# rpacheco-blazquez/PINN-FEM

Measured on AMD Instinct MI355X. Metric: element-residual-grad evals/sec (PINN+GD iteration: MLP fwd+bwd, stiffness, assembly, residual, Adam), collinear truss, higher is better.
Workload: dtype f32; 1 GPU; ex4 shape (nets (20, 15, 10), E and A evaluated), 1000000 elements per GPU, collinear 2-D truss h=1, alpha_data=100 with measurements at every node, load factor 0.1; elements_total=1000000, parallelism=elements sharded x1

## Files before the change

### include/pinnfem_hip.h

```cpp
#ifndef PINNFEM_HIP_H
#define PINNFEM_HIP_H

#include <stdint.h>

#ifdef __cplusplus
extern "C" {
#endif

#define PF_ABI_VERSION 7

#define PF_OK 0
#define PF_ERR_ARG (-1)
#define PF_ERR_UNSUPPORTED (-2)
#define PF_ERR_HIP (-3)

#define PF_DOF_FIXED 1u
#define PF_DOF_MEASURED 2u
#define PF_DOF_SHARED 4u
#define PF_DOF_GHOST 8u

#define PF_WG_SHUFFLE 0
#define PF_WG_MFMA 1
#define PF_WG_MFMA44 2
#define PF_WG_MFMA32 3
// ... 60 lines not shown
  int32_t n_tensors;
  int32_t wg_mode;
  float lam;
  float alpha_physics, alpha_data;
  float lr_u, lr_t;
  double tol;
  double beta1, beta2, eps;
  int32_t use_data;
  int32_t max_iter;
  float* theta_pad;
  float* prop_e;
  float* prop_a;
  float* g_f;
  float* g_ea;
  float* grad_u;
  float* grad_theta;
  float* partials;
  float* hist;
  pf_state* state;
  int32_t n_part_blocks;
  int32_t pad_total;
  const int32_t* pad_index;
  float n_meas_f;
  int32_t fe_mode;
  const int32_t* shared_dofs;
  const int32_t* shared_slot;
  int32_t n_shared;
  int32_t n_iface;
  int32_t own_lo, own_hi;
  int32_t part_half;
  int32_t prop_double;
  float* net_op;
  int32_t op_off[2];
  int32_t coord_exp;
  int32_t mlp_dtype;
  float* elem_k;
  float* theta_alt;
  float* u_alt;
  const int32_t* adj_other;
} pf_problem;

#define PF_MAX_BLOCKS 1024
#define PF_MAX_NODE_BLOCKS 4096
#define PF_NODE_SLOTS (PF_MAX_NODE_BLOCKS + 8)

int pf_abi_version(void);
const char* pf_last_error(void);
int pf_net_param_count(int in_dim, int width, int n_hidden);
int pf_padded_width(int width);
int pf_net_pad_count(int in_dim, int width, int n_hidden);
int pf_net_pad_index(int in_dim, int width, int n_hidden, int local);
int pf_sizeof(int what);
int pf_net_op_count(int in_dim, int width, int n_hidden);
long long pf_partials_count(const pf_problem* p);
#define PF_FUSED_FORWARD 1
#define PF_FUSED_BACKWARD 2
#define PF_FUSED_THETA_UPDATE 4
#define PF_FUSED_U_PINGPONG 8
#define PF_FUSED_U_UPDATE 16
int pf_fusion_info(const pf_problem* p);

int pf_pack_theta(const pf_problem* p, void* stream);
int pf_net_forward(const pf_problem* p, int which, void* stream);
int pf_net_forward_all(const pf_problem* p, void* stream);
int pf_net_backward_all(const pf_problem* p, void* stream);
int pf_internal_force(const pf_problem* p, const float* u, float* f_int_out, void* stream);
int pf_node_residual(const pf_problem* p, float* f_int_out, void* stream);
int pf_elem_adjoint(const pf_problem* p, void* stream);
int pf_net_backward(const pf_problem* p, int which, void* stream);
int pf_node_gradu(const pf_problem* p, int fuse_adam, void* stream);
int pf_theta_reduce(const pf_problem* p, int fuse_adam, void* stream);
int pf_finalize(const pf_problem* p, void* stream);
int pf_reset(const pf_problem* p, void* stream);

int pf_gd_iterations(const pf_problem* p, int n_iter, void* stream);
int pf_graph_create(const pf_problem* p, int iters_per_graph, void* stream, void** graph_out);
#define PF_GRAPH_CONT_HEAD 1
#define PF_GRAPH_NO_TAIL 2
int pf_graph_create_ex(const pf_problem* p, int iters_per_graph, int flags, void* stream, void** graph_out);
int pf_graph_tail(const pf_problem* p, int iters_per_graph, void* stream);
int pf_graph_launch(void* graph, void* stream);
int pf_graph_destroy(void* graph);
#define PF_KERNEL_SLOTS 9
int pf_gd_iterations_timed(const pf_problem* p, int n_iter, void* stream, float* ms_per_kernel);
int pf_loss_and_grads(const pf_problem* p, void* stream);

int pf_shard_forward(const pf_problem* p, void* stream);
int pf_shard_backward(const pf_problem* p, float* buf, const float* u2_local, void* stream);
int pf_shard_update_interior(const pf_problem* p, void* stream);
int pf_shard_update_shared(const pf_problem* p, const float* buf, float* u2_local, void* stream);
int pf_shard_flush(const pf_problem* p, const float* u2_reduced, void* stream);

#define PF_COMM_ID_BYTES 128
int pf_comm_unique_id(const char* librccl_path, void* id_out);
int pf_comm_create(const char* librccl_path, const void* id, int rank, int world, void** comm_out);
int pf_comm_destroy(void* comm);
int pf_comm_abort(void* comm);
int pf_comm_info(void* comm, int* rank_out, int* nranks_out);
int pf_comm_all_reduce(void* comm, float* buf, int n, void* stream);
int pf_shard_iterations(const pf_problem* p, void* comm, int n_iter, float* buf, float* u2_local, void* stream);
int pf_shard_graph_create(const pf_problem* p, void* comm, int iters_per_graph, float* buf, float* u2_local, void* stream,
                          void** graph_out);
int pf_shard_iterations_graph(const pf_problem* p, void* comm, void* graph, int iters_per_graph, int n_iter, float* buf,
                              float* u2_local, void* stream);

int pf_kv_f64(const pf_problem* p, const double* v, double* out, int zero_fixed, void* stream);
// ... 32 lines not shown
```

### pinn_fem_amd/_capi.py

```python
from __future__ import annotations

import ctypes as C
import os

_HERE = os.path.dirname(os.path.abspath(__file__))
LIB_PATH = os.environ.get("PINNFEM_LIB") or os.path.join(_HERE, "lib", "libpinnfem_hip.so")

PF_ABI_VERSION = 7
PF_OK, PF_ERR_ARG, PF_ERR_UNSUPPORTED, PF_ERR_HIP = 0, -1, -2, -3
PF_DOF_FIXED, PF_DOF_MEASURED, PF_DOF_SHARED, PF_DOF_GHOST = 1, 2, 4, 8
PF_WG_SHUFFLE, PF_WG_MFMA, PF_WG_MFMA44, PF_WG_MFMA32 = 0, 1, 2, 3
PF_N32_WIDTH_MAX = 30
PF_MLP_F32, PF_MLP_BF16 = 0, 1
PF_FE_REFERENCE, PF_FE_DELTA = 0, 1
PF_HIST_COLS = 6
PF_MAX_BLOCKS = 1024
PF_COMM_ID_BYTES = 128
PF_MAX_NODE_BLOCKS = 4096
PF_NODE_SLOTS = PF_MAX_NODE_BLOCKS + 8
PF_KERNEL_SLOTS = 9
PF_GRAPH_CONT_HEAD, PF_GRAPH_NO_TAIL = 1, 2
PF_FUSED_FORWARD, PF_FUSED_BACKWARD, PF_FUSED_THETA_UPDATE, PF_FUSED_U_PINGPONG, PF_FUSED_U_UPDATE = 1, 2, 4, 8, 16
KERNEL_SLOT_NAMES = ("net_forward_young", "net_forward_area", "node_residual", "elem_adjoint",
                     "net_backward_young", "net_backward_area", "node_gradu_adam", "theta_reduce_adam",
# ... 27 lines not shown
        ("_pad2", C.c_float),
        ("loss_total", C.c_float), ("loss_physics", C.c_float), ("loss_data", C.c_float),
        ("u_norm", C.c_float), ("residual_norm", C.c_float), ("theta_norm", C.c_float),
        ("u_half", C.c_int32), ("_pad3", C.c_float),
    ]


class PfProblem(C.Structure):
    _fields_ = [
        ("mesh", PfMesh), ("net", PfNet * 2),
        ("u", C.c_void_p), ("m_u", C.c_void_p), ("v_u", C.c_void_p),
        ("theta", C.c_void_p), ("m_t", C.c_void_p), ("v_t", C.c_void_p),
        ("n_theta", C.c_int32), ("n_theta_active", C.c_int32),
        ("tensor_off", C.c_void_p),
        ("n_tensors", C.c_int32), ("wg_mode", C.c_int32),
        ("lam", C.c_float), ("alpha_physics", C.c_float), ("alpha_data", C.c_float),
        ("lr_u", C.c_float), ("lr_t", C.c_float),
        ("tol", C.c_double), ("beta1", C.c_double), ("beta2", C.c_double), ("eps", C.c_double),
        ("use_data", C.c_int32), ("max_iter", C.c_int32),
        ("theta_pad", C.c_void_p), ("prop_e", C.c_void_p), ("prop_a", C.c_void_p),
        ("g_f", C.c_void_p), ("g_ea", C.c_void_p), ("grad_u", C.c_void_p),
        ("grad_theta", C.c_void_p), ("partials", C.c_void_p), ("hist", C.c_void_p),
        ("state", C.c_void_p),
        ("n_part_blocks", C.c_int32), ("pad_total", C.c_int32),
        ("pad_index", C.c_void_p),
        ("n_meas_f", C.c_float), ("fe_mode", C.c_int32),
        ("shared_dofs", C.c_void_p), ("shared_slot", C.c_void_p),
        ("n_shared", C.c_int32), ("n_iface", C.c_int32),
        ("own_lo", C.c_int32), ("own_hi", C.c_int32), ("part_half", C.c_int32), ("prop_double", C.c_int32),
        ("net_op", C.c_void_p), ("op_off", C.c_int32 * 2), ("coord_exp", C.c_int32), ("mlp_dtype", C.c_int32),
        ("elem_k", C.c_void_p), ("theta_alt", C.c_void_p), ("u_alt", C.c_void_p), ("adj_other", C.c_void_p),
    ]


class PfScalarId(C.Structure):
    _fields_ = [
        ("p", C.c_void_p), ("m_p", C.c_void_p), ("v_p", C.c_void_p), ("table", C.c_void_p),
        ("n_rows", C.c_int32), ("has_bounds", C.c_int32),
        ("lo", C.c_float * 2), ("hi", C.c_float * 2),
        ("inv_ea0", C.c_float), ("lr_p", C.c_float), ("n_free_f", C.c_float), ("_pad", C.c_float),
    ]


_PP = C.POINTER(PfProblem)
SYMBOLS = {
    "pf_abi_version": (C.c_int, []),
    "pf_last_error": (C.c_char_p, []),
    "pf_net_param_count": (C.c_int, [C.c_int, C.c_int, C.c_int]),
    "pf_padded_width": (C.c_int, [C.c_int]),
    "pf_net_pad_count": (C.c_int, [C.c_int, C.c_int, C.c_int]),
    "pf_net_pad_index": (C.c_int, [C.c_int, C.c_int, C.c_int, C.c_int]),
    "pf_sizeof": (C.c_int, [C.c_int]),
    "pf_net_op_count": (C.c_int, [C.c_int, C.c_int, C.c_int]),
    "pf_partials_count": (C.c_longlong, [_PP]),
    "pf_fusion_info": (C.c_int, [_PP]),
    "pf_pack_theta": (C.c_int, [_PP, C.c_void_p]),
    "pf_net_forward": (C.c_int, [_PP, C.c_int, C.c_void_p]),
    "pf_net_forward_all": (C.c_int, [_PP, C.c_void_p]),
    "pf_net_backward_all": (C.c_int, [_PP, C.c_void_p]),
    "pf_internal_force": (C.c_int, [_PP, C.c_void_p, C.c_void_p, C.c_void_p]),
    "pf_node_residual": (C.c_int, [_PP, C.c_void_p, C.c_void_p]),
    "pf_elem_adjoint": (C.c_int, [_PP, C.c_void_p]),
    "pf_net_backward": (C.c_int, [_PP, C.c_int, C.c_void_p]),
    "pf_node_gradu": (C.c_int, [_PP, C.c_int, C.c_void_p]),
    "pf_theta_reduce": (C.c_int, [_PP, C.c_int, C.c_void_p]),
    "pf_finalize": (C.c_int, [_PP, C.c_void_p]),
    "pf_reset": (C.c_int, [_PP, C.c_void_p]),
    "pf_gd_iterations": (C.c_int, [_PP, C.c_int, C.c_void_p]),
    "pf_graph_create": (C.c_int, [_PP, C.c_int, C.c_void_p, C.POINTER(C.c_void_p)]),
    "pf_graph_create_ex": (C.c_int, [_PP, C.c_int, C.c_int, C.c_void_p, C.POINTER(C.c_void_p)]),
    "pf_graph_tail": (C.c_int, [_PP, C.c_int, C.c_void_p]),
    "pf_graph_launch": (C.c_int, [C.c_void_p, C.c_void_p]),
    "pf_graph_destroy": (C.c_int, [C.c_void_p]),
    "pf_gd_iterations_timed": (C.c_int, [_PP, C.c_int, C.c_void_p, C.POINTER(C.c_float)]),
    "pf_loss_and_grads": (C.c_int, [_PP, C.c_void_p]),
    "pf_shard_forward": (C.c_int, [_PP, C.c_void_p]),
    "pf_shard_backward": (C.c_int, [_PP, C.c_void_p, C.c_void_p, C.c_void_p]),
    "pf_shard_flush": (C.c_int, [_PP, C.c_void_p, C.c_void_p]),
    "pf_shard_update_interior": (C.c_int, [_PP, C.c_void_p]),
    "pf_shard_update_shared": (C.c_int, [_PP, C.c_void_p, C.c_void_p, C.c_void_p]),
    "pf_kv_f64": (C.c_int, [_PP, C.c_void_p, C.c_void_p, C.c_int, C.c_void_p]),
    "pf_pcg_workspace_count": (C.c_longlong, [_PP]),
    "pf_pcg_begin": (C.c_int, [_PP, C.c_void_p, C.c_void_p, C.c_void_p, C.c_double, C.c_void_p]),
    "pf_pcg_iterations": (C.c_int, [_PP, C.c_void_p, C.c_void_p, C.c_int, C.POINTER(C.c_double), C.c_void_p]),
    "pf_pcg_graph_create": (C.c_int, [_PP, C.c_void_p, C.c_void_p, C.c_int, C.c_void_p, C.POINTER(C.c_void_p)]),
    "pf_pcg_state": (C.c_int, [_PP, C.c_void_p, C.POINTER(C.c_double), C.c_void_p]),
    "pf_comm_unique_id": (C.c_int, [C.c_char_p, C.c_void_p]),
    "pf_comm_create": (C.c_int, [C.c_char_p, C.c_void_p, C.c_int, C.c_int, C.POINTER(C.c_void_p)]),
    "pf_comm_destroy": (C.c_int, [C.c_void_p]),
    "pf_comm_abort": (C.c_int, [C.c_void_p]),
    "pf_comm_info": (C.c_int, [C.c_void_p, C.POINTER(C.c_int), C.POINTER(C.c_int)]),
    "pf_comm_all_reduce": (C.c_int, [C.c_void_p, C.c_void_p, C.c_int, C.c_void_p]),
    "pf_shard_iterations": (C.c_int, [_PP, C.c_void_p, C.c_int, C.c_void_p, C.c_void_p, C.c_void_p]),
    "pf_shard_graph_create": (C.c_int, [_PP, C.c_void_p, C.c_int, C.c_void_p, C.c_void_p, C.c_void_p,
                                        C.POINTER(C.c_void_p)]),
    "pf_shard_iterations_graph": (C.c_int, [_PP, C.c_void_p, C.c_void_p, C.c_int, C.c_int, C.c_void_p, C.c_void_p,
                                            C.c_void_p]),
    "pf_scalar_gd_iterations": (C.c_int, [_PP, C.POINTER(PfScalarId), C.c_int, C.c_void_p]),
    "pf_adam": (C.c_int, [C.c_void_p, C.c_void_p, C.c_void_p, C.c_void_p, C.c_int, C.c_int,
                          C.c_double, C.c_double, C.c_double, C.c_double, C.c_void_p]),
    "pf_diag_k": (C.c_int, [_PP, C.c_void_p, C.c_void_p]),
    "pf_dense_k": (C.c_int, [_PP, C.c_void_p, C.c_void_p]),
    "pf_coo_k": (C.c_int, [_PP, C.c_void_p, C.c_void_p, C.c_void_p, C.c_void_p]),
}


# ... 50 lines not shown
```

### pinn_fem_amd/csrc/pf_api.hip

```cpp
#include <stdlib.h>
#include <string.h>
#include <stdio.h>
#include "pf_common.h"
#include "pf_net32.h"

int pf_launch_node_residual(const pf_problem* p, float* f_int_out, int compute_loss, hipStream_t s, int fin_prev = 0);
int pf_launch_elem_adjoint(const pf_problem* p, hipStream_t s);
int pf_launch_node_gradu(const pf_problem* p, int fuse_adam, hipStream_t s, int skip_shared = 0, float* u_out = nullptr);
int pf_launch_u_home(const pf_problem* p, hipStream_t s);
int pf_launch_scalar_residual(const pf_problem* p, const pf_scalar_id* sp, hipStream_t s);
int pf_launch_scalar_update(const pf_problem* p, const pf_scalar_id* sp, hipStream_t s);
int pf_launch_shard_pack(const pf_problem* p, float* buf2, const float* u2_local, hipStream_t s);
int pf_launch_shard_update(const pf_problem* p, const float* buf2, float* u2_local, hipStream_t s);
int pf_launch_shard_flush(const pf_problem* p, const float* u2, hipStream_t s);
int pf_launch_theta_reduce(const pf_problem* p, int fuse_adam, hipStream_t s);
int pf_launch_pack_theta(const pf_problem* p, hipStream_t s);
int pf_launch_finalize(const pf_problem* p, int mode, int with_theta, hipStream_t s, int tn_ready = 0);
int pf_launch_theta_stage1(const pf_problem* p, hipStream_t s);
int pf_launch_theta_stage2(const pf_problem* p, int fuse_adam, hipStream_t s);
int pf_launch_reset(const pf_problem* p, hipStream_t s);
int pf_launch_adam(float* param, const float* grad, float* m, float* v, int n, int step, double lr,
                   double beta1, double beta2, double eps, hipStream_t s);
int pf_launch_diag_k(const pf_problem* p, float* diag, hipStream_t s);
int pf_launch_dense_k(const pf_problem* p, float* K, hipStream_t s);
// ... 212 lines not shown

int pf_abi_version(void) { return PF_ABI_VERSION; }
const char* pf_last_error(void) { return g_err; }

int pf_sizeof(int what) {
  switch (what) {
    case 0: return (int)sizeof(pf_mesh);
    case 1: return (int)sizeof(pf_net);
    case 2: return (int)sizeof(pf_state);
    case 3: return (int)sizeof(pf_problem);
    case 4: return (int)sizeof(pf_scalar_id);
  }
  return PF_ERR_ARG;
}

int pf_net_param_count(int in_dim, int width, int n_hidden) {
  if (in_dim < 1 || width < 1 || n_hidden < 1) return PF_ERR_ARG;
  return width * in_dim + width + (n_hidden - 1) * (width * width + width) + width + 1;
}

int pf_padded_width(int width) { return padded_width(width); }

int pf_net_pad_count(int in_dim, int width, int n_hidden) {
  const int hp = padded_width(width);
  if (hp < 0 || n_hidden < 1 || n_hidden > 3 || (in_dim != 2 && in_dim != 3)) return PF_ERR_UNSUPPORTED;
  return pf_pad_count(hp, n_hidden);
}

int pf_net_pad_index(int in_dim, int width, int n_hidden, int local) {
  const int hp = padded_width(width);
  if (hp < 0 || n_hidden < 1 || n_hidden > 3 || (in_dim != 2 && in_dim != 3)) return PF_ERR_UNSUPPORTED;
  int q = local;
  if (q < 0) return PF_ERR_ARG;
  if (q < width * in_dim) return (q / in_dim) * 4 + (q % in_dim);
  q -= width * in_dim;
  if (q < width) return q * 4 + in_dim;
  q -= width;
  for (int l = 2; l <= n_hidden; ++l) {
    if (q < width * width) return pf_pad_wh(hp, l) + (q / width) * (hp + 4) + (q % width);
    q -= width * width;
    if (q < width) return pf_pad_wh(hp, l) + q * (hp + 4) + hp;
    q -= width;
  }
  if (q < width) return pf_pad_wo(hp, n_hidden) + q;
  q -= width;
  if (q == 0) return pf_pad_wo(hp, n_hidden) + hp;
  return PF_ERR_ARG;
}

int pf_net_op_count(int in_dim, int width, int n_hidden) {
  if (width < 1 || width > PF_N32_WIDTH_MAX || n_hidden < 1 || n_hidden > 3 || (in_dim != 2 && in_dim != 3))
    return PF_ERR_UNSUPPORTED;
  return (pf_n32_bytes(n_hidden) + 3) / 4;
}

long long pf_partials_count(const pf_problem* p) {
  if (!p) return PF_ERR_ARG;
  return (long long)PF_PART_WG + ((long long)p->n_part_blocks + PF_RG) * (long long)p->pad_total;
}

int pf_fusion_info(const pf_problem* p) {
  if (check_problem(p) != PF_OK) return PF_ERR_ARG;
  int m = 0;
  if (can_fuse_forward(p)) m |= PF_FUSED_FORWARD;
  if (can_fuse_backward(p)) m |= PF_FUSED_BACKWARD;
  if (can_fuse_theta_update(p)) m |= PF_FUSED_THETA_UPDATE;
  if (p->prop_double != 0 && p->elem_k != nullptr && can_fuse_gradu(p)) m |= PF_FUSED_U_UPDATE;
  else if (p->u_alt != nullptr && p->mesh.n_elems >= PF_GRAPH_DAG_MIN_ELEMS) m |= PF_FUSED_U_PINGPONG;
  return m;
}

int pf_pack_theta(const pf_problem* p, void* stream) {
  int rc = check_problem(p);
  if (rc) return rc;
  PF_TRY(pf_launch_pack_theta(p, (hipStream_t)stream), "pf_pack_theta");
  return PF_OK;
}

int pf_net_forward(const pf_problem* p, int which, void* stream) {
  int rc = check_problem(p);
  if (rc) return rc;
  if (which < 0 || which > 1 || !p->net[which].enabled) return fail(PF_ERR_ARG, "net not enabled");
  PF_TRY(net_forward(p, which, (hipStream_t)stream), "pf_net_forward");
  return PF_OK;
}

int pf_net_forward_all(const pf_problem* p, void* stream) {
  int rc = check_problem(p);
  if (rc) return rc;
  PF_TRY(net_forward_all(p, (hipStream_t)stream), "pf_net_forward_all");
  return PF_OK;
}

int pf_net_backward_all(const pf_problem* p, void* stream) {
  int rc = check_problem(p);
  if (rc) return rc;
  if (!(p->net[0].enabled || p->net[1].enabled)) return PF_OK;
  return enqueue_backwards(p, (hipStream_t)stream);
}

int pf_internal_force(const pf_problem* p, const float* u, float* f_int_out, void* stream) {
  int rc = check_problem(p);
  if (rc) return rc;
  if (!u || !f_int_out) return fail(PF_ERR_ARG, "null u / f_int_out");
  pf_problem q = *p;
  q.u = const_cast<float*>(u);
// ... 502 lines not shown
```

### pinn_fem_amd/csrc/pf_net32.h

```cpp
#pragma once
#include "pf_common.h"

#define PF_N32_MAX_WIDTH 30
#define PF_N32_KA 2048.0f
#define PF_N32_KW 16.0f
#define PF_N32_KB 16.0f
__host__ __device__ inline float pf_n32_lam_scale(float lam) {
  const float a = lam < 0.f ? -lam : lam;
  if (!(a > 0.f) || !(a < 3.0e38f)) return 1.0f;
  int ex = 0;
  (void)frexpf(a, &ex);
  ex = ex < -100 ? -100 : ex;
  return ldexpf(1.0f, 14 - ex);
}

__host__ __device__ constexpr int pf_n32_off_w1() { return 16; }
__host__ __device__ constexpr int pf_n32_off_wo() { return 16 + 512; }
__host__ __device__ constexpr int pf_n32_off_bo() { return 16 + 512 + 128; }
__host__ __device__ constexpr int pf_n32_off_layers() { return 16 + 512 + 128 + 16; }
#define PF_N32_LAYER_BYTES (128 + 4096 + 4096)
__host__ __device__ constexpr int pf_n32_off_bias(int l) { return pf_n32_off_layers() + (l - 2) * PF_N32_LAYER_BYTES; }
__host__ __device__ constexpr int pf_n32_off_af(int l) { return pf_n32_off_bias(l) + 128; }
__host__ __device__ constexpr int pf_n32_off_ab(int l) { return pf_n32_off_af(l) + 4096; }
__host__ __device__ constexpr int pf_n32_bytes(int n_hidden) { return pf_n32_off_layers() + (n_hidden - 1) * PF_N32_LAYER_BYTES; }
// ... 37 lines not shown
      unsigned short hf[8], hb[8];
#pragma unroll
      for (int j = 0; j < 8; ++j) {
        const int u_k = 2 * (8 * ks + j) + hh;
        float vf = 0.f, vb = 0.f;
        if (u_row < W && u_k < W) {
          vf = PF_N32_KW * Wl[u_row * W + u_k];
          vb = PF_N32_KB * Wl[u_k * W + u_row];
        }
        if (prec == 1) {
          hf[j] = sp ? (unsigned short)0 : __builtin_bit_cast(unsigned short, (__bf16)vf);
          hb[j] = sp ? (unsigned short)0 : __builtin_bit_cast(unsigned short, (__bf16)vb);
        } else {
          const _Float16 fh = (_Float16)vf, bh = (_Float16)vb;
          hf[j] = __builtin_bit_cast(unsigned short, sp ? (_Float16)(vf - (float)fh) : fh);
          hb[j] = __builtin_bit_cast(unsigned short, sp ? (_Float16)(vb - (float)bh) : bh);
        }
      }
      af[i] = make_uint4(hf[0] | (unsigned)hf[1] << 16, hf[2] | (unsigned)hf[3] << 16, hf[4] | (unsigned)hf[5] << 16,
                         hf[6] | (unsigned)hf[7] << 16);
      ab[i] = make_uint4(hb[0] | (unsigned)hb[1] << 16, hb[2] | (unsigned)hb[3] << 16, hb[4] | (unsigned)hb[5] << 16,
                         hb[6] | (unsigned)hb[7] << 16);
    }
  }
  if (with_bound && (tid >> 6) == ((nt - 1) >> 6)) {
    const int lane = tid & 63;
    float v = lane < W ? fabsf(th[o_wo + lane]) : 0.f;
    float bound = 0.f, grow = 1.f;
    for (int l = L; l >= 1; --l) {
      float m = v;
#pragma unroll
      for (int d = 32; d >= 1; d >>= 1) m = fmaxf(m, __shfl_xor(m, d));
      bound = fmaxf(bound, grow * m);
      grow *= 4.f;
      if (l >= 2) {
        const float* Wl = th + o_h + (l - 2) * per;
        float a = 0.f;
#pragma unroll 4
        for (int j = 0; j < W; ++j) {
          const float w = lane < W ? fabsf(Wl[j * W + lane]) : 0.f;
          a += w * __shfl(v, j);
        }
        v = a;
      }
    }
    if (lane == 0) {
      float* hdr = reinterpret_cast<float*>(img);
      hdr[0] = bound > 0.f ? bound : 1.f;
      hdr[1] = hdr[2] = hdr[3] = 0.f;
    }
  }
}

#define PF_FWD32_MAX_BLOCKS 256
inline int pf_n32_fwd2_blocks(int n_elems) {
  int nb = (n_elems + 1023) / 1024;
  if (nb > PF_FWD32_MAX_BLOCKS) nb = PF_FWD32_MAX_BLOCKS;
  if (nb < 1) nb = 1;
  return nb;
}
#define PF_GU_M 2
inline bool pf_n32_fwd2_can_update_u(const pf_problem* p, int gu_nb) {
  if (!p->adj_other || !p->m_u || !p->v_u || p->mesh.n_elems <= 0) return false;
  if (p->n_shared != 0 || p->own_lo != 0 || p->own_hi != 0) return false;
  const int nb = pf_n32_fwd2_blocks(p->mesh.n_elems);
  if (nb > gu_nb) return false;
  const int ntasks = (p->mesh.n_nodes + 64 * PF_GU_M - 1) / (64 * PF_GU_M);
  return (ntasks + nb - 1) / nb <= 1024 - 16;
}
```

### pinn_fem_amd/csrc/pf_net32.hip

```cpp
#include <type_traits>
#include <stdlib.h>
#include "pf_net32.h"
#include "pf_node.h"

#ifndef PF_NR
#error "compile with -DPF_NR=<registers per lane>"
#endif
#ifndef PF_PREC
#define PF_PREC 0
#endif
#ifndef PF_N32_DBG_ENABLE
#define PF_N32_DBG_ENABLE 0
#endif
#define PF_CAT2(a, b) a##b
#define PF_CAT(a, b) PF_CAT2(a, b)

typedef _Float16 h2 __attribute__((ext_vector_type(2)));
typedef _Float16 h8 __attribute__((ext_vector_type(8)));
typedef short s4v __attribute__((ext_vector_type(4)));
typedef float f32x16 __attribute__((ext_vector_type(16)));
typedef unsigned u32x4 __attribute__((ext_vector_type(4)));
typedef unsigned u32x2 __attribute__((ext_vector_type(2)));
typedef __bf16 bf2 __attribute__((ext_vector_type(2)));
typedef __bf16 bf8 __attribute__((ext_vector_type(8)));
// ... 909 lines not shown
__device__ __forceinline__ void bw_row_from_parked(const pf_problem& P, int which, int hp, const float* __restrict__ park,
                                                   float kl, float kx) {
  const pf_net net = P.net[which];
  const int waves = blockDim.x >> 6, W = net.width;
  constexpr int PS = bw_park_floats<L>();
  float* __restrict__ prow = P.partials + PF_PART_WG + (size_t)blockIdx.x * P.pad_total + net.pad_off;
  const int padc = pf_pad_count(hp, L);
  for (int i = threadIdx.x; i < padc; i += blockDim.x) prow[i] = 0.f;
  __syncthreads();
  sfor<0, L>([&](auto l) {
    constexpr int LL = l + 1;
    float sc = 1.f;
    for (int k = 0; k < L - LL; ++k) sc *= 4.f;
    for (int idx = threadIdx.x; idx < 1024; idx += blockDim.x) {
      const int m = idx >> 5, c = idx & 31;
      const int j = 2 * (m & 15) + (m >> 4);
      if ((m & 15) >= NR || j >= W) continue;
      float t = 0.f;
      for (int q = 0; q < waves; ++q) t += park[q * PS + (LL - 1) * 1024 + idx];
      int dst = -1;
      float k = sc;
      if (LL >= 2) {
        const int kk = 2 * (c & 15) + (c >> 4);
        k *= PF_N32_KA;
        if (c == 15) dst = pf_pad_wh(hp, LL) + j * (hp + 4) + hp;
        else if ((c & 15) < NR && kk < W) dst = pf_pad_wh(hp, LL) + j * (hp + 4) + kk;
      } else {
        if (c < IN) { dst = j * 4 + c; k *= c == 0 ? kl : kx; }
        else if (c == IN) dst = j * 4 + IN;
      }
      if (dst >= 0) prow[dst] = t / k;
    }
  });
  float* const pwo = prow + pf_pad_wo(hp, L);
  if (threadIdx.x < 32) {
    const int hh = threadIdx.x >> 4, r = threadIdx.x & 15, u = 2 * r + hh;
    if (r < NR && u < W) {
      float t = 0.f;
      for (int q = 0; q < waves; ++q) t += park[q * PS + L * 1024 + hh * 16 + r];
      pwo[u] = t * (1.0f / PF_N32_KA);
    }
  }
  if (threadIdx.x == 32) {
    float t = 0.f;
    for (int q = 0; q < waves; ++q) t += park[q * PS + L * 1024 + 32];
    pwo[hp] = t;
  }
}

template <int NR, int L, int IN, bool GEA, int MODE = 0, class FirstRow = int>
__device__ __forceinline__ void backward_phase(const pf_problem& P, int which, int hp, int dbg, const unsigned char* smem,
                                               unsigned char* cst, unsigned char* wscr,
                                               unsigned long long* stamps = nullptr, float* park = nullptr,
                                               FirstRow first_row = FirstRow(), int shift8 = 0) {
  using E = Eng<NR>;
  constexpr int CONST_BYTES = E::CONST_BYTES, WAVE_SCRATCH = E::WAVE_SCRATCH, REGION = E::REGION, NPK = E::NPK;
  constexpr bool COMPACT = E::COMPACT;
  typedef typename E::WriteBase WriteBase;
  constexpr int DIM = IN - 1;
  const pf_net net = P.net[which];
  const pf_net onet = P.net[1 - which];
  const float* __restrict__ other = which == 0 ? P.prop_a : P.prop_e;
  const float* __restrict__ mine = which == 0 ? P.prop_e : P.prop_a;
  const int n = P.mesh.n_elems;
  const int lane = threadIdx.x & 63, wv = threadIdx.x >> 6, waves = blockDim.x >> 6;
  const int h = lane >> 5;
  unsigned char* scratch = wscr + wv * WAVE_SCRATCH;
  if constexpr (MODE != 2)
    for (int i = threadIdx.x; i < CONST_BYTES / 4; i += blockDim.x) reinterpret_cast<unsigned*>(cst)[i] = 0u;
  for (int i = lane; i < WAVE_SCRATCH / 16; i += 64) reinterpret_cast<uint4*>(scratch)[i] = make_uint4(0, 0, 0, 0);
  if constexpr (MODE != 2) __syncthreads();
  if (MODE != 2 && threadIdx.x < 32)
    if constexpr (COMPACT)
      *reinterpret_cast<unsigned short*>(cst + 192 + REGION + 64 * (threadIdx.x >> 2) + 8 * (threadIdx.x & 3) + 6) = BF ? 0x4500 : 0x6800;
  const unsigned char* rd = E::operand_base(scratch, lane, cst + 192);
  const WriteBase wb = E::write_base(scratch, lane);

  const int per_round = (int)gridDim.x * waves;
  const int ntasks_all = (n + 63) >> 6;
  const int slot = (int)blockIdx.x * waves + wv;
  const int hw = waves >> 1;
  const bool elder = wv < hw;
  const int partner = elder ? slot + hw : slot - hw;
  const int c_own = slot < ntasks_all ? (ntasks_all - 1 - slot) / per_round + 1 : 0;
  const int c_par = (hw > 0 && partner < ntasks_all) ? (ntasks_all - 1 - partner) / per_round + 1 : 0;
  const int sh = min((shift8 > 0 && hw > 0 && (waves & 1) == 0) ? (((elder ? c_par : c_own) * shift8 + 4) >> 3) : 0,
                     elder ? c_par : c_own);
  const int n_mine = elder ? c_own + sh : c_own - sh;
  auto task_base = [&](int k) {
    if (k < (elder ? c_own : n_mine)) return (k * per_round + slot) * 64;
    if (elder && k < n_mine) return ((c_par - sh + (k - c_own)) * per_round + partner) * 64;
    return n - 1;
  };
  TaskIn<DIM> nxt;
  int2 nn_ahead = int2{0, 0};
  if (n > 0) {
    task_fetch_a<IN, GEA>(nxt, P, onet, other, mine, min(task_base(0) + lane, n - 1));
    if (GEA) nn_ahead = reinterpret_cast<const int2*>(P.mesh.conn)[min(task_base(1) + lane, n - 1)];
  }
  if constexpr (MODE != 2) __syncthreads();
  task_fetch_b<IN, GEA>(nxt, P);

  const float bound = __builtin_bit_cast(float, __builtin_amdgcn_readfirstlane(__builtin_bit_cast(int, reinterpret_cast<const float*>(smem)[0])));
  const float kx = __builtin_bit_cast(float, __builtin_amdgcn_readfirstlane(__builtin_bit_cast(int, __builtin_ldexpf(1.0f, P.coord_exp))));
  const float inv_scale = __builtin_bit_cast(float, __builtin_amdgcn_readfirstlane(__builtin_bit_cast(int, 1.0f / net.scale)));
  const float kl = __builtin_bit_cast(float, __builtin_amdgcn_readfirstlane(__builtin_bit_cast(int, pf_n32_lam_scale(P.lam))));
  f32x16 T[L];
  sfor<0, L>([&](auto l) { constexpr int LL = l; T[LL] = zero16(); });
  float Srun = 0.f;
  float go[NR];
  sfor<0, NR>([&](auto r) { constexpr int R = r; go[R] = 0.f; });
  float gbo = 0.f;

  if (PF_N32_DBG_ENABLE && stamps) stamps[0] = __builtin_amdgcn_s_memrealtime();
  for (int k = 0; k < n_mine; ++k) {
    const int base = task_base(k);
    const int e = base + lane;
    const bool live = e < n;
    const TaskIn<DIM> cur = nxt;
    const bool more = k + 1 < n_mine;
    float gz = 0.f;
    if (live) {
      float gea;
      if (GEA) {
        gea = task_gea<DIM>(cur, P.fe_mode);
        P.g_ea[e] = gea;
      } else {
        gea = cur.gea;
      }
      float g = gea * cur.oth;
      g = g * net.scale;
      gz = net.positive ? g * one_minus_exp_neg(cur.own * inv_scale) : g;
    }
    const float gabs = fabsf(gz) * bound;
    if (Srun == 0.f || __builtin_amdgcn_ballot_w64(gabs * Srun >= 16384.0f) != 0ull) {
      const float gmax = wave_max(gabs);
      if (gmax > 0.f && gmax < 3.0e38f) {
        int ex = 0;
        (void)frexpf(gmax, &ex);
        ex = ex < -100 ? -100 : (ex > 100 ? 100 : ex);
        const float Sneed = __builtin_ldexpf(1.0f, 14 - ex);
        if (Srun == 0.f) Srun = Sneed;
        else if (Sneed < Srun) {
          const float f = Sneed / Srun;
          sfor<0, L>([&](auto l) {
            constexpr int LL = l;
            sfor<0, 16>([&](auto i) { constexpr int I = i; T[LL][I] *= f; });
          });
          Srun = Sneed;
        }
      }
    }
    const float S = Srun == 0.f ? 1.0f : Srun;
    float g0, g1;
    both_tiles(gz, g0, g1);
    float xa0, xa1, xb0, xb1;
    both_tiles(cur.x[1], xa0, xa1);
    both_tiles(cur.x[2], xb0, xb1);
    const float lam_in = cur.x[0];
    if (more) {
      task_fetch_a<IN, GEA>(nxt, P, onet, other, mine, min(task_base(k + 1) + lane, n - 1), false);
      if (GEA) {
        nxt.nn = nn_ahead;
        task_fetch_b<IN, GEA>(nxt, P);
        nn_ahead = reinterpret_cast<const int2*>(P.mesh.conn)[min(task_base(k + 2) + lane, n - 1)];
      }
    }
    auto tile_backward = [&](const typename E::template TileAct<L, true>& A, const float (&xt)[3], float gt, bool go_done) {
      unsigned xhi[NPK], xlo[NPK];
      sfor<2, NPK>([&](auto q) { constexpr int Q = q; xhi[Q] = 0u; xlo[Q] = 0u; });
      split_pair(kl * xt[0], kx * xt[1], xhi[0], xlo[0]);
      split_pair(IN == 3 ? kx * xt[2] : 1.0f, IN == 3 ? 1.0f : 0.f, xhi[1], xlo[1]);
      if (!go_done) sfor<0, NR>([&](auto r) { constexpr int R = r; go[R] = fmaf(gt, A.aL[R], go[R]); });
      if (!(dbg & 2)) E::template backward_tile<L, IN>(smem, scratch, lane, A, gt * S, xhi, xlo, T, wb, rd, dbg);
    };
    if constexpr (E::template bw_pair<L>()) {
      const float x0[3] = {lam_in, xa0, xb0}, x1[3] = {lam_in, xa1, xb1};
      typename E::template TileAct<L, true> A0, A1;
      float p0, p1;
      E::template forward_tiles<L, IN, true>(smem, lane, x0, x1, A0, A1, p0, p1, 0, -1, go, g0, g1);
      tile_backward(A0, x0, g0, true);
      tile_backward(A1, x1, g1, true);
    } else {
      sfor<0, 2>([&](auto tt) {
        constexpr int TT = tt;
        const float xt[3] = {lam_in, TT ? xa1 : xa0, TT ? xb1 : xb0};
        typename E::template TileAct<L, true> A;
        E::template recompute_tile<L, IN>(smem, lane, xt, A);
        tile_backward(A, xt, TT ? g1 : g0, false);
      });
    }
    gbo += gz;
  }
  if (PF_N32_DBG_ENABLE && stamps) stamps[1] = __builtin_amdgcn_s_memrealtime();
  const float invS = Srun == 0.f ? 1.0f : 1.0f / Srun;
  sfor<0, L>([&](auto l) {
    constexpr int LL = l;
    sfor<0, 16>([&](auto i) { constexpr int I = i; T[LL][I] *= invS; });
  });
  if constexpr (MODE == 1) {
    bw_park<NR, L>(park + (size_t)wv * bw_park_floats<L>(), T, go, gbo, lane);
    if (PF_N32_DBG_ENABLE && stamps) stamps[2] = __builtin_amdgcn_s_memrealtime();
    return;
  } else if constexpr (MODE == 2) {
    __syncthreads();
    first_row();
    __syncthreads();
    bw_park<NR, L>(park + (size_t)wv * bw_park_floats<L>(), T, go, gbo, lane);
    __syncthreads();
    bw_row_from_parked<NR, L, IN>(P, which, hp, park, kl, kx);
    if (PF_N32_DBG_ENABLE && stamps) stamps[2] = __builtin_amdgcn_s_memrealtime();
    return;
  }

  __syncthreads();
  float* stage = reinterpret_cast<float*>(wscr);
  const int W = net.width;
  float* __restrict__ prow = P.partials + PF_PART_WG + (size_t)blockIdx.x * P.pad_total + net.pad_off;
  const int padc = pf_pad_count(hp, L);
  for (int i = threadIdx.x; i < padc; i += blockDim.x) prow[i] = 0.f;
  sfor<0, L>([&](auto l) {
    constexpr int LL = l + 1;
    __syncthreads();
    sfor<0, 16>([&](auto i) {
      constexpr int I = i;
      const int m = (I & 3) + 8 * (I >> 2) + 4 * h;
      stage[wv * 1024 + m * 32 + (lane & 31)] = T[LL - 1][I];
    });
    __syncthreads();
    float sc = 1.f;
    for (int k = 0; k < L - LL; ++k) sc *= 4.f;
    for (int idx = threadIdx.x; idx < 1024; idx += blockDim.x) {
      const int m = idx >> 5, c = idx & 31;
      const int j = 2 * (m & 15) + (m >> 4);
      if ((m & 15) >= NR || j >= W) continue;
      float t = 0.f;
      for (int q = 0; q < waves; ++q) t += stage[q * 1024 + idx];
      int dst = -1;
      float k = sc;
      if (LL >= 2) {
        const int kk = 2 * (c & 15) + (c >> 4);
        k *= PF_N32_KA;
        if (c == 15) dst = pf_pad_wh(hp, LL) + j * (hp + 4) + hp;
        else if ((c & 15) < NR && kk < W) dst = pf_pad_wh(hp, LL) + j * (hp + 4) + kk;
      } else {
        if (c < IN) { dst = j * 4 + c; k *= c == 0 ? kl : kx; }
        else if (c == IN) dst = j * 4 + IN;
      }
      if (dst >= 0) prow[dst] = t / k;
    }
  });
  __syncthreads();
  sfor<0, NR>([&](auto r) {
    constexpr int R = r;
    float v = go[R];
#pragma unroll
    for (int o = 16; o > 0; o >>= 1) v += __shfl_xor(v, o, 64);
    if ((lane & 31) == 0) stage[wv * 64 + h * 16 + R] = v;
  });
  {
    const float v = pf_wave_sum(gbo);
    if (lane == 0) stage[waves * 64 + wv] = v;
  }
  __syncthreads();
  float* const pwo = prow + pf_pad_wo(hp, L);
  if (threadIdx.x < 32) {
    const int hh = threadIdx.x >> 4, r = threadIdx.x & 15, u = 2 * r + hh;
    if (r < NR && u < W) {
      float t = 0.f;
      for (int q = 0; q < waves; ++q) t += stage[q * 64 + hh * 16 + r];
      pwo[u] = t * (1.0f / PF_N32_KA);
    }
  }
  if (threadIdx.x == 32) {
    float t = 0.f;
    for (int q = 0; q < waves; ++q) t += stage[waves * 64 + q];
    pwo[hp] = t;
  }
  if (PF_N32_DBG_ENABLE && stamps) stamps[2] = __builtin_amdgcn_s_memrealtime();
}


template <int NR, int L, int IN, bool GEA>
__global__ __launch_bounds__((Eng<NR>::template bw_threads<L, GEA>())) void k_net32_backward(pf_problem P, int which, int hp, int dbg_arg) {
  using E = Eng<NR>;
  const int dbg = PF_N32_DBG_ENABLE ? dbg_arg : 0;
  extern __shared__ __align__(16) unsigned char smem[];
  constexpr int IMG = pf_n32_bytes(L), IMGPAD = (IMG + 255) & ~255;
  __shared__ int s_done;
  if (threadIdx.x == 0) s_done = P.state->done;
  copy_image(smem, reinterpret_cast<const unsigned char*>(P.net_op + P.op_off[which]), IMG);
  __syncthreads();
  if (s_done != 0 || P.mesh.n_elems <= 0) return;
  backward_phase<NR, L, IN, GEA>(P, which, hp, dbg, smem, smem + IMGPAD, smem + IMGPAD + E::CONST_BYTES);
}

template <int NRE, int NRA, int L, int IN>
constexpr int bw2_threads() {
  return Eng<NRE>::template bw_threads<L, true>() < Eng<NRA>::template bw_threads<L, false>()
             ? Eng<NRE>::template bw_threads<L, true>() : Eng<NRA>::template bw_threads<L, false>();
}
template <int NRE, int NRA>
constexpr int bw2_const_bytes() { return Eng<NRE>::CONST_BYTES > Eng<NRA>::CONST_BYTES ? Eng<NRE>::CONST_BYTES : Eng<NRA>::CONST_BYTES; }
template <int NRE, int NRA>
constexpr int bw2_wave_scratch() { return Eng<NRE>::WAVE_SCRATCH > Eng<NRA>::WAVE_SCRATCH ? Eng<NRE>::WAVE_SCRATCH : Eng<NRA>::WAVE_SCRATCH; }

template <int NRE, int NRA>
constexpr bool bw2_parked() { return Eng<NRE>::COMPACT && Eng<NRA>::COMPACT; }
template <int NRE, int NRA, int L, int IN>
constexpr size_t bw2_lds_bytes() {
  return 2 * (size_t)((pf_n32_bytes(L) + 255) & ~255) + bw2_const_bytes<NRE, NRA>() +
         (size_t)(bw2_threads<NRE, NRA, L, IN>() / 64) * bw2_wave_scratch<NRE, NRA>() +
         (bw2_parked<NRE, NRA>() ? (size_t)(bw2_threads<NRE, NRA, L, IN>() / 64) * bw_park_floats<L>() * sizeof(float) : 0);
}
constexpr int PF_BW_SHIFT = 2;
template <int NRE, int NRA, int L, int IN>
__global__ __launch_bounds__((bw2_threads<NRE, NRA, L, IN>())) void k_net32_backward2(pf_problem P, int hp_e, int hp_a, int dbg_arg) {
  const int dbg = PF_N32_DBG_ENABLE ? dbg_arg : 0;
  const unsigned long long t_entry = PF_N32_DBG_ENABLE ? __builtin_amdgcn_s_memrealtime() : 0ull;
  extern __shared__ __align__(16) unsigned char smem[];
  constexpr int IMG = pf_n32_bytes(L), IMGPAD = (IMG + 255) & ~255;
  __shared__ int s_done;
  if (threadIdx.x == 0) s_done = P.state->done;
  copy_images2(smem, reinterpret_cast<const unsigned char*>(P.net_op + P.op_off[0]), smem + IMGPAD,
               reinterpret_cast<const unsigned char*>(P.net_op + P.op_off[1]), IMG);
  __syncthreads();
  if (s_done != 0 || P.mesh.n_elems <= 0) return;
  unsigned char* cst = smem + 2 * IMGPAD;
  unsigned char* wscr = cst + bw2_const_bytes<NRE, NRA>();
  unsigned long long* st = nullptr;
  if (PF_N32_DBG_ENABLE && (dbg & 16) && (threadIdx.x & 63) == 0) {
    st = reinterpret_cast<unsigned long long*>(P.u_alt) + 65536 + (size_t)(blockIdx.x * (blockDim.x >> 6) + (threadIdx.x >> 6)) * 8;
    st[0] = t_entry;
  }
  if constexpr (bw2_parked<NRE, NRA>()) {
    float* park = reinterpret_cast<float*>(wscr + (size_t)(blockDim.x >> 6) * bw2_wave_scratch<NRE, NRA>());
    const float kl_e = pf_n32_lam_scale(P.lam), kx_e = __builtin_ldexpf(1.0f, P.coord_exp);
    auto first_row = [&]() { bw_row_from_parked<NRE, L, IN>(P, 0, hp_e, park, kl_e, kx_e); };
    backward_phase<NRE, L, IN, true, 1>(P, 0, hp_e, dbg, smem, cst, wscr, st ? st + 1 : nullptr, park, 0, PF_BW_SHIFT);
    backward_phase<NRA, L, IN, false, 2>(P, 1, hp_a, dbg, smem + IMGPAD, cst, wscr, st ? st + 4 : nullptr, park, first_row,
                                         PF_BW_SHIFT);
  } else {
    backward_phase<NRE, L, IN, true>(P, 0, hp_e, dbg, smem, cst, wscr, st ? st + 1 : nullptr, nullptr, 0, PF_BW_SHIFT);
    __syncthreads();
    backward_phase<NRA, L, IN, false>(P, 1, hp_a, dbg, smem + IMGPAD, cst, wscr, st ? st + 4 : nullptr, nullptr, 0, PF_BW_SHIFT);
  }
}

template <int L, int IN>
int launch_fwd(const pf_problem* p, int which, hipStream_t s, int s2_half) {
  constexpr int NR = PF_NR;
  const int nb = pf_n32_fwd2_blocks(p->mesh.n_elems);
  static const int dbg = getenv("PF_N32_DBG") ? atoi(getenv("PF_N32_DBG")) : 0;
  const int ws = p->elem_k != nullptr ? 1 : 0;
  const size_t lds = s2_half < 0 ? (size_t)pf_n32_bytes(L)
                                 : (size_t)((pf_n32_bytes(L) + 255) & ~255) + (size_t)p->n_theta_active * sizeof(float);
  if (lds > 64000) { pf_set_error("too many trainable parameters for the fused theta update"); return PF_ERR_UNSUPPORTED; }
  hipLaunchKernelGGL((k_net32_forward<NR, L, IN>), dim3(nb), dim3(FW_THREADS), lds, s, *p, which, dbg, ws, s2_half);
  return hipGetLastError() == hipSuccess ? PF_OK : PF_ERR_HIP;
}

template <int L, int IN, bool GEA>
int launch_bwd_t(const pf_problem* p, int which, hipStream_t s) {
  const int nb = pf_net_blocks(p);
  const int hp = ((p->net[which].width + 3) / 4) * 4;
  constexpr int NR = PF_NR;
  using E = Eng<NR>;
  constexpr int BW_THREADS = E::template bw_threads<L, GEA>();
  const size_t lds = ((pf_n32_bytes(L) + 255) & ~255) + E::CONST_BYTES + (size_t)(BW_THREADS / 64) * E::WAVE_SCRATCH;
  static_assert(E::WAVE_SCRATCH >= 4096 + 512, "write-out staging must fit the wave scratch");
  static const int dbg = getenv("PF_N32_DBG") ? atoi(getenv("PF_N32_DBG")) : 0;
  hipLaunchKernelGGL((k_net32_backward<NR, L, IN, GEA>), dim3(nb), dim3(BW_THREADS), lds, s, *p, which, hp, dbg);
  return hipGetLastError() == hipSuccess ? PF_OK : PF_ERR_HIP;
}
template <int L, int IN>
int launch_bwd(const pf_problem* p, int which, hipStream_t s) { return launch_bwd_t<L, IN, false>(p, which, s); }
template <int L, int IN>
int launch_bwd_gea(const pf_problem* p, int which, hipStream_t s) { return launch_bwd_t<L, IN, true>(p, which, s); }

template <int NRA, int L, int IN>
int launch_fwd2_t(const pf_problem* p, hipStream_t s, const pf_fwd2_opts& o) {
  const int s2_half = o.s2_half, gu_nb = o.gu_nb;
  constexpr int NRE = PF_NR;
  const int n = p->mesh.n_elems;
  const int nb = pf_n32_fwd2_blocks(n);
  static const int dbg = getenv("PF_N32_DBG") ? atoi(getenv("PF_N32_DBG")) : 0;
  const size_t lds = 2 * (size_t)((pf_n32_bytes(L) + 255) & ~255) + (s2_half < 0 ? 0 : (size_t)p->n_theta_active * sizeof(float));
  if (lds > 64000) { pf_set_error("too many trainable parameters for the fused theta update"); return PF_ERR_UNSUPPORTED; }
  if (gu_nb > 0 && !pf_n32_fwd2_can_update_u(p, gu_nb)) { pf_set_error("fused forward: displacement update not possible on this problem"); return PF_ERR_UNSUPPORTED; }
  hipLaunchKernelGGL((k_net32_forward2<NRE, NRA, L, IN>), dim3(nb), dim3(FW_THREADS), lds, s, *p, dbg, s2_half >= 0 && o.calc_index ? s2_half + 2 : s2_half, gu_nb, o.gu_k);
  return hipGetLastError() == hipSuccess ? PF_OK : PF_ERR_HIP;
}
template <int L, int IN>
int launch_fwd2(const pf_problem* p, hipStream_t s, const pf_fwd2_opts& o) {
  switch (pf_net32_bucket(p->net[1].width)) {
    case 2: return launch_fwd2_t<2, L, IN>(p, s, o);
    case 4: return launch_fwd2_t<4, L, IN>(p, s, o);
    case 6: return launch_fwd2_t<6, L, IN>(p, s, o);
// ... 109 lines not shown
```

Before: 7.660 billion element-evals/s.

## Rebalance backward MLP work between paired waves with fine-grained 32-element partition

Replaces the old per-wave task shift in the backward MLP kernel with a new partition walk. It splits leftover tiles at 32-element granularity and gives elder waves a tunable share (38/64) of each wave pair's work, adding a half-tile single entry where needed. The goal is to even out load between paired waves, whose tile costs differ, and to shorten the tail. The cost is more index arithmetic per task, a separate code path for half-wave single tiles, and risk of ordering or coverage errors in the intricate partition maths. A host-callable walk function is exported so the partition can be checked.

Result: no change. 7.616 billion element-evals/s (-0.6%).

```diff
diff --git a/include/pinnfem_hip.h b/include/pinnfem_hip.h
--- a/include/pinnfem_hip.h
+++ b/include/pinnfem_hip.h
@@ -136,6 +136,7 @@
 int pf_net_pad_index(int in_dim, int width, int n_hidden, int local);
 int pf_sizeof(int what);
 int pf_net_op_count(int in_dim, int width, int n_hidden);
+int pf_bw_partition_walk(int n_elems, int blocks, int waves, int slot, int* bases, int* tiles, int cap);
 long long pf_partials_count(const pf_problem* p);
 #define PF_FUSED_FORWARD 1
 #define PF_FUSED_BACKWARD 2
diff --git a/pinn_fem_amd/_capi.py b/pinn_fem_amd/_capi.py
--- a/pinn_fem_amd/_capi.py
+++ b/pinn_fem_amd/_capi.py
@@ -103,6 +103,8 @@
     "pf_net_pad_index": (C.c_int, [C.c_int, C.c_int, C.c_int, C.c_int]),
     "pf_sizeof": (C.c_int, [C.c_int]),
     "pf_net_op_count": (C.c_int, [C.c_int, C.c_int, C.c_int]),
+    "pf_bw_partition_walk": (C.c_int, [C.c_int, C.c_int, C.c_int, C.c_int, C.POINTER(C.c_int), C.POINTER(C.c_int),
+                                       C.c_int]),
     "pf_partials_count": (C.c_longlong, [_PP]),
     "pf_fusion_info": (C.c_int, [_PP]),
     "pf_pack_theta": (C.c_int, [_PP, C.c_void_p]),
diff --git a/pinn_fem_amd/csrc/pf_api.hip b/pinn_fem_amd/csrc/pf_api.hip
--- a/pinn_fem_amd/csrc/pf_api.hip
+++ b/pinn_fem_amd/csrc/pf_api.hip
@@ -288,6 +288,18 @@
   if (width < 1 || width > PF_N32_WIDTH_MAX || n_hidden < 1 || n_hidden > 3 || (in_dim != 2 && in_dim != 3))
     return PF_ERR_UNSUPPORTED;
   return (pf_n32_bytes(n_hidden) + 3) / 4;
+}
+
+int pf_bw_partition_walk(int n_elems, int blocks, int waves, int slot, int* bases, int* tiles, int cap) {
+  if (n_elems < 0 || blocks < 1 || waves < 1 || slot < 0 || slot >= blocks * waves || cap < 0 || (cap > 0 && (!bases || !tiles)))
+    return fail(PF_ERR_ARG, "pf_bw_partition_walk: bad argument");
+  const pf_bw_walk w = pf_bw_partition(n_elems, blocks, waves, slot);
+  const int n = w.n_whole + (w.single >= 0 ? 1 : 0);
+  for (int k = 0; k < n && k < cap; ++k) {
+    bases[k] = pf_bw_entry(w, k);
+    tiles[k] = k < w.n_whole ? 2 : 1;
+  }
+  return n;
 }
 
 long long pf_partials_count(const pf_problem* p) {
diff --git a/pinn_fem_amd/csrc/pf_net32.h b/pinn_fem_amd/csrc/pf_net32.h
--- a/pinn_fem_amd/csrc/pf_net32.h
+++ b/pinn_fem_amd/csrc/pf_net32.h
@@ -113,6 +113,74 @@
   }
 }
 
+#define PF_BW_ELDER_DEN 64
+#ifndef PF_BW_ELDER_NUM
+#define PF_BW_ELDER_NUM 38
+#endif
+struct pf_bw_walk {
+  int n_whole;
+  int single;
+  int col;
+  int lead;
+  int inter_end;
+  int partner;
+  int per_round;
+  int chunk0;
+};
+__host__ __device__ inline pf_bw_walk pf_bw_partition(int n_elems, int blocks, int waves, int slot,
+                                                      int elder_num = PF_BW_ELDER_NUM) {
+  pf_bw_walk w;
+  const int per_round = blocks * waves;
+  const int ntasks = (n_elems + 63) >> 6, nt = (n_elems + 31) >> 5;
+  w.single = -1; w.col = slot; w.partner = slot; w.per_round = per_round; w.chunk0 = 0;
+  if (ntasks <= per_round || (waves & 1)) {
+    w.n_whole = slot < ntasks ? (ntasks - 1 - slot) / per_round + 1 : 0;
+    w.lead = w.inter_end = w.n_whole;
+    return w;
+  }
+  const int hw = waves >> 1, wv = slot % waves;
+  const bool elder = wv < hw;
+  const int pairs = blocks * hw, p = (slot / waves) * hw + (elder ? wv : wv - hw);
+  const int R = nt / (2 * per_round), rem = nt - R * 2 * per_round;
+  const int qb = rem / pairs, qr = rem % pairs;
+  const int q = qb + (p < qr ? 1 : 0);
+  const int chunk = (R * per_round) * 64 + (p * qb + (p < qr ? p : qr)) * 32;
+  const int t = 4 * R + q;
+  int e = (t * elder_num + PF_BW_ELDER_DEN / 2) / PF_BW_ELDER_DEN;
+  e = e < 2 * R ? 2 * R : (e > t ? t : e);
+  const int y = t - e;
+  const int ycount = R + (q >> 1);
+  const bool split = !(q & 1) && (y & 1);
+  const int s0 = y >> 1;
+  const int ylast = (ycount - 1 < R) ? ((ycount - 1) * per_round + slot + (elder ? hw : 0)) * 64
+                                     : chunk + (ycount - 1 - R) * 64;
+  if (!elder) {
+    w.n_whole = s0;
+    w.lead = w.inter_end = s0 < R ? s0 : R;
+    w.chunk0 = chunk;
+    if (y & 1) w.single = split ? ylast : chunk + (q >> 1) * 64;
+  } else {
+    w.partner = slot + hw;
+    w.lead = s0 < R ? s0 : R;
+    w.inter_end = w.lead + 2 * (R - w.lead);
+    const int from = s0 > R ? s0 : R;
+    w.chunk0 = chunk + (from - R) * 64;
+    if (split && ycount == R) w.inter_end -= 1;
+    w.n_whole = w.inter_end + (split && ycount == R ? 0 : ycount - (split ? 1 : 0) - from);
+    if (e & 1) w.single = split ? ylast + 32 : chunk + (q >> 1) * 64;
+  }
+  return w;
+}
+__host__ __device__ inline int pf_bw_entry(const pf_bw_walk& w, int k) {
+  if (k < w.lead) return (k * w.per_round + w.col) * 64;
+  if (k < w.inter_end) {
+    const int m = k - w.lead;
+    return ((w.lead + (m >> 1)) * w.per_round + ((m & 1) ? w.partner : w.col)) * 64;
+  }
+  if (k < w.n_whole) return w.chunk0 + (k - w.inter_end) * 64;
+  return k == w.n_whole ? w.single : -1;
+}
+
 #define PF_FWD32_MAX_BLOCKS 256
 inline int pf_n32_fwd2_blocks(int n_elems) {
   int nb = (n_elems + 1023) / 1024;
diff --git a/pinn_fem_amd/csrc/pf_net32.hip b/pinn_fem_amd/csrc/pf_net32.hip
--- a/pinn_fem_amd/csrc/pf_net32.hip
+++ b/pinn_fem_amd/csrc/pf_net32.hip
@@ -985,7 +985,7 @@
 __device__ __forceinline__ void backward_phase(const pf_problem& P, int which, int hp, int dbg, const unsigned char* smem,
                                                unsigned char* cst, unsigned char* wscr,
                                                unsigned long long* stamps = nullptr, float* park = nullptr,
-                                               FirstRow first_row = FirstRow(), int shift8 = 0) {
+                                               FirstRow first_row = FirstRow(), int elder_num = PF_BW_ELDER_NUM) {
   using E = Eng<NR>;
   constexpr int CONST_BYTES = E::CONST_BYTES, WAVE_SCRATCH = E::WAVE_SCRATCH, REGION = E::REGION, NPK = E::NPK;
   constexpr bool COMPACT = E::COMPACT;
@@ -1009,27 +1009,18 @@
   const unsigned char* rd = E::operand_base(scratch, lane, cst + 192);
   const WriteBase wb = E::write_base(scratch, lane);
 
-  const int per_round = (int)gridDim.x * waves;
-  const int ntasks_all = (n + 63) >> 6;
-  const int slot = (int)blockIdx.x * waves + wv;
-  const int hw = waves >> 1;
-  const bool elder = wv < hw;
-  const int partner = elder ? slot + hw : slot - hw;
-  const int c_own = slot < ntasks_all ? (ntasks_all - 1 - slot) / per_round + 1 : 0;
-  const int c_par = (hw > 0 && partner < ntasks_all) ? (ntasks_all - 1 - partner) / per_round + 1 : 0;
-  const int sh = min((shift8 > 0 && hw > 0 && (waves & 1) == 0) ? (((elder ? c_par : c_own) * shift8 + 4) >> 3) : 0,
-                     elder ? c_par : c_own);
-  const int n_mine = elder ? c_own + sh : c_own - sh;
-  auto task_base = [&](int k) {
-    if (k < (elder ? c_own : n_mine)) return (k * per_round + slot) * 64;
-    if (elder && k < n_mine) return ((c_par - sh + (k - c_own)) * per_round + partner) * 64;
-    return n - 1;
+  const pf_bw_walk walk = pf_bw_partition(n, (int)gridDim.x, waves, (int)blockIdx.x * waves + __builtin_amdgcn_readfirstlane(wv),
+                                          elder_num);
+  const int n_whole = walk.n_whole;
+  auto task_elem = [&](int k) {
+    const int b = pf_bw_entry(walk, k);
+    return b < 0 ? n - 1 : min(b + (k < n_whole ? lane : (lane & 31)), n - 1);
   };
   TaskIn<DIM> nxt;
   int2 nn_ahead = int2{0, 0};
   if (n > 0) {
-    task_fetch_a<IN, GEA>(nxt, P, onet, other, mine, min(task_base(0) + lane, n - 1));
-    if (GEA) nn_ahead = reinterpret_cast<const int2*>(P.mesh.conn)[min(task_base(1) + lane, n - 1)];
+    task_fetch_a<IN, GEA>(nxt, P, onet, other, mine, task_elem(0));
+    if (GEA) nn_ahead = reinterpret_cast<const int2*>(P.mesh.conn)[task_elem(1)];
   }
   if constexpr (MODE != 2) __syncthreads();
   task_fetch_b<IN, GEA>(nxt, P);
@@ -1046,12 +1037,13 @@
   float gbo = 0.f;
 
   if (PF_N32_DBG_ENABLE && stamps) stamps[0] = __builtin_amdgcn_s_memrealtime();
-  for (int k = 0; k < n_mine; ++k) {
-    const int base = task_base(k);
-    const int e = base + lane;
-    const bool live = e < n;
+  const int n_ent = n_whole + (walk.single >= 0 ? 1 : 0);
+  auto entry = [&](auto single_c, int k) {
+    constexpr bool SINGLE = decltype(single_c)::value;
+    const int e = pf_bw_entry(walk, k) + (SINGLE ? (lane & 31) : lane);
+    const bool live = e < n && !(SINGLE && lane >= 32);
     const TaskIn<DIM> cur = nxt;
-    const bool more = k + 1 < n_mine;
+    const bool more = !SINGLE && k + 1 < n_ent;
     float gz = 0.f;
     if (live) {
       float gea;
@@ -1092,11 +1084,11 @@
     both_tiles(cur.x[2], xb0, xb1);
     const float lam_in = cur.x[0];
     if (more) {
-      task_fetch_a<IN, GEA>(nxt, P, onet, other, mine, min(task_base(k + 1) + lane, n - 1), false);
+      task_fetch_a<IN, GEA>(nxt, P, onet, other, mine, task_elem(k + 1), false);
       if (GEA) {
         nxt.nn = nn_ahead;
         task_fetch_b<IN, GEA>(nxt, P);
-        nn_ahead = reinterpret_cast<const int2*>(P.mesh.conn)[min(task_base(k + 2) + lane, n - 1)];
+        nn_ahead = reinterpret_cast<const int2*>(P.mesh.conn)[task_elem(k + 2)];
       }
     }
     auto tile_backward = [&](const typename E::template TileAct<L, true>& A, const float (&xt)[3], float gt, bool go_done) {
@@ -1107,7 +1099,12 @@
       if (!go_done) sfor<0, NR>([&](auto r) { constexpr int R = r; go[R] = fmaf(gt, A.aL[R], go[R]); });
       if (!(dbg & 2)) E::template backward_tile<L, IN>(smem, scratch, lane, A, gt * S, xhi, xlo, T, wb, rd, dbg);
     };
-    if constexpr (E::template bw_pair<L>()) {
+    if constexpr (SINGLE) {
+      const float xt[3] = {lam_in, xa0, xb0};
+      typename E::template TileAct<L, true> A;
+      E::template recompute_tile<L, IN>(smem, lane, xt, A);
+      tile_backward(A, xt, g0, false);
+    } else if constexpr (E::template bw_pair<L>()) {
       const float x0[3] = {lam_in, xa0, xb0}, x1[3] = {lam_in, xa1, xb1};
       typename E::template TileAct<L, true> A0, A1;
       float p0, p1;
@@ -1124,7 +1121,9 @@
       });
     }
     gbo += gz;
-  }
+  };
+  for (int k = 0; k < n_whole; ++k) entry(std::false_type{}, k);
+  if (walk.single >= 0) entry(std::true_type{}, n_whole);
   if (PF_N32_DBG_ENABLE && stamps) stamps[1] = __builtin_amdgcn_s_memrealtime();
   const float invS = Srun == 0.f ? 1.0f : 1.0f / Srun;
   sfor<0, L>([&](auto l) {
@@ -1214,6 +1213,10 @@
 }
 
 
+__device__ __forceinline__ int bw_elder_num(int dbg) {
+  return PF_N32_DBG_ENABLE && ((dbg >> 8) & 127) ? (dbg >> 8) & 127 : PF_BW_ELDER_NUM;
+}
+
 template <int NR, int L, int IN, bool GEA>
 __global__ __launch_bounds__((Eng<NR>::template bw_threads<L, GEA>())) void k_net32_backward(pf_problem P, int which, int hp, int dbg_arg) {
   using E = Eng<NR>;
@@ -1225,7 +1228,8 @@
   copy_image(smem, reinterpret_cast<const unsigned char*>(P.net_op + P.op_off[which]), IMG);
   __syncthreads();
   if (s_done != 0 || P.mesh.n_elems <= 0) return;
-  backward_phase<NR, L, IN, GEA>(P, which, hp, dbg, smem, smem + IMGPAD, smem + IMGPAD + E::CONST_BYTES);
+  backward_phase<NR, L, IN, GEA>(P, which, hp, dbg, smem, smem + IMGPAD, smem + IMGPAD + E::CONST_BYTES, nullptr, nullptr, 0,
+                                 bw_elder_num(dbg));
 }
 
 template <int NRE, int NRA, int L, int IN>
@@ -1246,7 +1250,6 @@
          (size_t)(bw2_threads<NRE, NRA, L, IN>() / 64) * bw2_wave_scratch<NRE, NRA>() +
          (bw2_parked<NRE, NRA>() ? (size_t)(bw2_threads<NRE, NRA, L, IN>() / 64) * bw_park_floats<L>() * sizeof(float) : 0);
 }
-constexpr int PF_BW_SHIFT = 2;
 template <int NRE, int NRA, int L, int IN>
 __global__ __launch_bounds__((bw2_threads<NRE, NRA, L, IN>())) void k_net32_backward2(pf_problem P, int hp_e, int hp_a, int dbg_arg) {
   const int dbg = PF_N32_DBG_ENABLE ? dbg_arg : 0;
@@ -1266,17 +1269,17 @@
     st = reinterpret_cast<unsigned long long*>(P.u_alt) + 65536 + (size_t)(blockIdx.x * (blockDim.x >> 6) + (threadIdx.x >> 6)) * 8;
     st[0] = t_entry;
   }
+  const int en = bw_elder_num(dbg);
   if constexpr (bw2_parked<NRE, NRA>()) {
     float* park = reinterpret_cast<float*>(wscr + (size_t)(blockDim.x >> 6) * bw2_wave_scratch<NRE, NRA>());
     const float kl_e = pf_n32_lam_scale(P.lam), kx_e = __builtin_ldexpf(1.0f, P.coord_exp);
     auto first_row = [&]() { bw_row_from_parked<NRE, L, IN>(P, 0, hp_e, park, kl_e, kx_e); };
-    backward_phase<NRE, L, IN, true, 1>(P, 0, hp_e, dbg, smem, cst, wscr, st ? st + 1 : nullptr, park, 0, PF_BW_SHIFT);
-    backward_phase<NRA, L, IN, false, 2>(P, 1, hp_a, dbg, smem + IMGPAD, cst, wscr, st ? st + 4 : nullptr, park, first_row,
-                                         PF_BW_SHIFT);
+    backward_phase<NRE, L, IN, true, 1>(P, 0, hp_e, dbg, smem, cst, wscr, st ? st + 1 : nullptr, park, 0, en);
+    backward_phase<NRA, L, IN, false, 2>(P, 1, hp_a, dbg, smem + IMGPAD, cst, wscr, st ? st + 4 : nullptr, park, first_row, en);
   } else {
-    backward_phase<NRE, L, IN, true>(P, 0, hp_e, dbg, smem, cst, wscr, st ? st + 1 : nullptr, nullptr, 0, PF_BW_SHIFT);
+    backward_phase<NRE, L, IN, true>(P, 0, hp_e, dbg, smem, cst, wscr, st ? st + 1 : nullptr, nullptr, 0, en);
     __syncthreads();
-    backward_phase<NRA, L, IN, false>(P, 1, hp_a, dbg, smem + IMGPAD, cst, wscr, st ? st + 4 : nullptr, nullptr, 0, PF_BW_SHIFT);
+    backward_phase<NRA, L, IN, false>(P, 1, hp_a, dbg, smem + IMGPAD, cst, wscr, st ? st + 4 : nullptr, nullptr, 0, en);
   }
 }
 
```
